# JdeRobot/slam-SDVL

Hardware: AMD Instinct MI355X
Metric: tracked frames/sec (640x480, 5-lvl pyr, ~200 feats) (higher is better)
Workload: dtype u8/f32/f64

## Files before the change

### slam-sdvl_amd/csrc/sdvl_detect.hip

```cpp
#include <atomic>

#include "sdvl_internal.h"
#include "sdvl_wave.h"

namespace {

constexpr int kPyrTW = 32, kPyrTH = 8;

struct PyrJob {
  const uint8_t *src;
  uint8_t *dst;
  int sw, sh, dw, dh;
};

__device__ __forceinline__ int reflect101_clamped(int p, int n) {
  if (p < 0) p = -p;
  if (p >= n) p = 2 * n - 2 - p;
  return min(max(p, 0), n - 1);
}

template <int kPyrTW, int kPyrTH>
__global__ __launch_bounds__(kPyrTW * kPyrTH / 4) void pyr_down_kernel(const PyrJob *__restrict__ jobs, int n_jobs, int gx, int gy) {
  constexpr int kThreads = kPyrTW * kPyrTH / 4;
  constexpr int kPyrSH = 2 * kPyrTH + 3;
  constexpr int kPyrSWW = kPyrTW / 2 + 2;
  constexpr int kPyrPitch = (kPyrSWW + 1) * 4;
  const auto sync = [] {
    if (kThreads == 64) wave_sync();
    else __syncthreads();
  };
  __shared__ uint32_t s_srcw[kPyrSH * (kPyrSWW + 1)];
  __shared__ __attribute__((aligned(8))) uint16_t s_h[kPyrSH][kPyrTW];
  const int id = blockIdx.x, per_frame = gx * gy;
  const int slot = id >> 3;
  const int bz = (slot / per_frame) * 8 + (id & 7);
  if (bz >= n_jobs) return;
  const int tq = slot % per_frame;
  const int by = tq / gx, bx = tq - by * gx;
  const PyrJob job = jobs[bz];
  const int tx0 = bx * kPyrTW, ty0 = by * kPyrTH;
  if (tx0 >= job.dw || ty0 >= job.dh) return;
  const int tid = threadIdx.x;
  uint8_t *s_bytes = reinterpret_cast<uint8_t *>(s_srcw);
  const int xb = 2 * tx0 - 4;
  const int nx = min(kPyrTW, job.dw - tx0), ny = min(kPyrTH, job.dh - ty0);
  const int rows = 2 * ny + 3, last_byte = 2 * nx + 4;
  if ((job.sw & 3) == 0 && (reinterpret_cast<uintptr_t>(job.src) & 3u) == 0) {
    const int words_row = job.sw >> 2, w0 = xb >> 2;
    const int nwords = last_byte / 4 + 1;
    constexpr int kRowLanes = (kPyrSWW + 3) / 4, kRowsPerRound = kThreads / kRowLanes;
    if (words_row >= 4) {
      const int lr = tid / kRowLanes, lq = tid - lr * kRowLanes;
      const int first = w0 + 4 * lq;
      const int s = min(max(first, 0), words_row - 4);
      const int col0 = s - w0;
      if (lr < kRowsPerRound && 4 * lq < nwords) {
        for (int r = lr; r < rows; r += kRowsPerRound) {
          const int sy = reflect101_clamped(2 * ty0 - 2 + r, job.sh);
          const __attribute__((address_space(1))) uint32_t *srcw = (const __attribute__((address_space(1))) uint32_t *)job.src;
          const __attribute__((address_space(1))) uint32_t *pw = srcw + static_cast<uint32_t>(sy * words_row + s);
          const uint32_t v[4] = {pw[0], pw[1], pw[2], pw[3]};
          uint32_t *dst = &s_srcw[r * (kPyrSWW + 1)];
#pragma unroll
          for (int k = 0; k < 4; k++) {
            const int c = col0 + k;
            if (c >= 0 && c < nwords) dst[c] = v[k];
          }
        }
      }
    } else
    for (int idx = tid; idx < rows * kPyrSWW; idx += kThreads) {
      const int r = idx / kPyrSWW, c = idx - r * kPyrSWW;
      if (c >= nwords) continue;
      const int sy = reflect101_clamped(2 * ty0 - 2 + r, job.sh);
      const int wi = min(max(w0 + c, 0), words_row - 1);
      s_srcw[r * (kPyrSWW + 1) + c] = reinterpret_cast<const uint32_t *>(job.src + static_cast<size_t>(sy) * job.sw)[wi];
    }
    sync();
    if (tid < rows && (xb < 0 || xb + last_byte >= job.sw)) {
      uint8_t *row = s_bytes + tid * kPyrPitch;
      if (xb < 0) {
        row[2] = row[6];
        row[3] = row[5];
      }
      for (int b = max(2, job.sw - xb); b <= last_byte; b++) row[b] = row[max(reflect101_clamped(xb + b, job.sw) - xb, 0)];
    }
  } else {
    const int ncols = last_byte - 1;
    for (int idx = tid; idx < rows * ncols; idx += kThreads) {
      const int r = idx / ncols, c = idx - r * ncols;
      const int sy = reflect101_clamped(2 * ty0 - 2 + r, job.sh);
      const int sx = reflect101_clamped(2 * tx0 - 2 + c, job.sw);
      s_bytes[r * kPyrPitch + 2 + c] = job.src[static_cast<size_t>(sy) * job.sw + sx];
    }
  }
  sync();
  typedef unsigned short u16x2 __attribute__((ext_vector_type(2)));
  for (int idx = tid; idx < rows * (kPyrTW / 2); idx += kThreads) {
    const int r = idx / (kPyrTW / 2), xp = idx - r * (kPyrTW / 2);
    if (2 * xp < nx) {
      const uint32_t *w = &s_srcw[r * (kPyrSWW + 1) + xp];
      const uint32_t w0 = w[0], w1 = w[1], w2 = w[2];
      const uint32_t hx = __builtin_amdgcn_udot4(w1, 0x00010406u, __builtin_amdgcn_udot4(w0, 0x04010000u, 0u, false), false);
      const uint32_t hx1 = __builtin_amdgcn_udot4(w2, 0x00000001u, __builtin_amdgcn_udot4(w1, 0x04060401u, 0u, false), false);
      const uint32_t h = hx | (hx1 << 16);
      *reinterpret_cast<uint32_t *>(&s_h[r][2 * xp]) = __builtin_bit_cast(uint32_t, h);
    }
  }
  sync();
  {
    const int y = tid / (kPyrTW / 4), x = (tid % (kPyrTW / 4)) * 4;
    const int oy = ty0 + y, ox = tx0 + x;
    if (oy < job.dh && ox < job.dw) {
      u16x2 a01 = {0, 0}, a23 = {0, 0};
#pragma unroll
      for (int t = 0; t < 5; t++) {
        const unsigned short wg = (t == 0 || t == 4) ? 1 : (t == 2 ? 6 : 4);
        const u16x2 wgt = {wg, wg};
        const uint2 hv = *reinterpret_cast<const uint2 *>(&s_h[2 * y + t][x]);
        a01 += wgt * __builtin_bit_cast(u16x2, hv.x);
        a23 += wgt * __builtin_bit_cast(u16x2, hv.y);
      }
      const u16x2 half = {128, 128};
      a01 = (a01 + half) >> 8;
      a23 = (a23 + half) >> 8;
      int acc[4] = {a01.x, a01.y, a23.x, a23.y};
      uint8_t *d = job.dst + static_cast<size_t>(oy) * job.dw + ox;
      if (ox + 3 < job.dw && (reinterpret_cast<uintptr_t>(job.dst) & 3u) == 0 && (job.dw & 3) == 0) {
        __attribute__((address_space(1))) uint32_t *dstw = (__attribute__((address_space(1))) uint32_t *)job.dst;
        dstw[static_cast<uint32_t>(oy * job.dw + ox) >> 2] = __builtin_amdgcn_perm(__builtin_bit_cast(uint32_t, a23), __builtin_bit_cast(uint32_t, a01), 0x06040200u);
      } else {
#pragma unroll
        for (int k = 0; k < 4; k++)
          if (ox + k < job.dw) d[k] = static_cast<uint8_t>(acc[k]);
      }
    }
  }
}

struct FastLevels {
  int n_levels;
  int cell_begin[SDVL_MAX_LEVELS + 1];
  int wcells[SDVL_MAX_LEVELS];
  int cell_size, margin, threshold;
  int dense_num;
};

struct __attribute__((aligned(16))) CellGeo {
  uint32_t xy;
  uint32_t wh;
  int32_t level;
  int32_t pair_inv;
};

struct FastJob {
  const uint8_t *level[4];
  int lw[4], lh[4];
  uint32_t *cell_kps;
  int32_t *cell_counts;
};


constexpr int kTile = 32;
constexpr int kPitchW = 12;
constexpr int kPadRows = 3;

__device__ __forceinline__ bool ring_run9(uint32_t m) {
  const uint32_t M = m | (m << 16);
  uint32_t r = M & (M >> 1);
  r &= (r >> 2);
  r &= (r >> 4);
  r &= (M >> 8);
  return (r & 0xFFFFu) != 0;
}

__device__ __forceinline__ int byte_of(uint32_t w0, uint32_t w1, uint32_t w2, int i) {
  return static_cast<int>(((i < 4 ? w0 : (i < 8 ? w1 : w2)) >> (8 * (i & 3))) & 0xFFu);
}

__device__ __forceinline__ bool fast_compass_pass(int v, int p_dn, int p_rt, int p_up, int p_lf, int t) {
  const int hi = v + t, lo = v - t;
  const bool b0 = p_dn > hi, b4 = p_rt > hi, b8 = p_up > hi, b12 = p_lf > hi;
  const bool d0 = p_dn < lo, d4 = p_rt < lo, d8 = p_up < lo, d12 = p_lf < lo;
  return (b0 && b4) || (b4 && b8) || (b8 && b12) || (b12 && b0) || (d0 && d4) || (d4 && d8) || (d8 && d12) || (d12 && d0);
}

#define SDVL_MIN2(a, b) min((a), (b))
#define SDVL_MAX2(a, b) max((a), (b))

__device__ __forceinline__ int fast_corner_best(const uint8_t *tile, int pitch_bytes, int t) {
  const int v = tile[0];
#define SDVL_E(K, DX, DY) const int e##K = static_cast<int>(tile[(DY) * pitch_bytes + (DX)]);
  SDVL_E(0, 0, 3) SDVL_E(1, 1, 3) SDVL_E(2, 2, 2) SDVL_E(3, 3, 1) SDVL_E(4, 3, 0) SDVL_E(5, 3, -1) SDVL_E(6, 2, -2) SDVL_E(7, 1, -3)
  SDVL_E(8, 0, -3) SDVL_E(9, -1, -3) SDVL_E(10, -2, -2) SDVL_E(11, -3, -1) SDVL_E(12, -3, 0) SDVL_E(13, -3, 1) SDVL_E(14, -2, 2) SDVL_E(15, -1, 3)
#undef SDVL_E
#define SDVL_MIN3(a, b, c) min(min((a), (b)), (c))
#define SDVL_MAX3(a, b, c) max(max((a), (b)), (c))
#define SDVL_W3(K, A, B, C) const int n##K = SDVL_MIN3(e##A, e##B, e##C), x##K = SDVL_MAX3(e##A, e##B, e##C);
  SDVL_W3(0, 0, 1, 2) SDVL_W3(1, 1, 2, 3) SDVL_W3(2, 2, 3, 4) SDVL_W3(3, 3, 4, 5) SDVL_W3(4, 4, 5, 6) SDVL_W3(5, 5, 6, 7)
  SDVL_W3(6, 6, 7, 8) SDVL_W3(7, 7, 8, 9) SDVL_W3(8, 8, 9, 10) SDVL_W3(9, 9, 10, 11) SDVL_W3(10, 10, 11, 12) SDVL_W3(11, 11, 12, 13)
  SDVL_W3(12, 12, 13, 14) SDVL_W3(13, 13, 14, 15) SDVL_W3(14, 14, 15, 0) SDVL_W3(15, 15, 0, 1)
#undef SDVL_W3
#define SDVL_W9(K, A, B, C) const int N##K = SDVL_MIN3(n##A, n##B, n##C), X##K = SDVL_MAX3(x##A, x##B, x##C);
  SDVL_W9(0, 0, 3, 6) SDVL_W9(1, 1, 4, 7) SDVL_W9(2, 2, 5, 8) SDVL_W9(3, 3, 6, 9) SDVL_W9(4, 4, 7, 10) SDVL_W9(5, 5, 8, 11)
  SDVL_W9(6, 6, 9, 12) SDVL_W9(7, 7, 10, 13) SDVL_W9(8, 8, 11, 14) SDVL_W9(9, 9, 12, 15) SDVL_W9(10, 10, 13, 0) SDVL_W9(11, 11, 14, 1)
  SDVL_W9(12, 12, 15, 2) SDVL_W9(13, 13, 0, 3) SDVL_W9(14, 14, 1, 4) SDVL_W9(15, 15, 2, 5)
#undef SDVL_W9
  const int max_n = SDVL_MAX3(SDVL_MAX3(N0, N1, N2), SDVL_MAX3(N3, N4, N5), SDVL_MAX3(SDVL_MAX3(N6, N7, N8), SDVL_MAX3(N9, N10, N11), SDVL_MAX3(N12, N13, SDVL_MAX2(N14, N15))));
  const int min_x = SDVL_MIN3(SDVL_MIN3(X0, X1, X2), SDVL_MIN3(X3, X4, X5), SDVL_MIN3(SDVL_MIN3(X6, X7, X8), SDVL_MIN3(X9, X10, X11), SDVL_MIN3(X12, X13, SDVL_MIN2(X14, X15))));
#undef SDVL_MIN3
#undef SDVL_MAX3
  return max(max(t, v - min_x), max_n - v);
}


constexpr int kPitchHW = 20;

typedef _Float16 h2 __attribute__((ext_vector_type(2)));
__device__ __forceinline__ h2 pk_min3(h2 a, h2 b, h2 c) {
  h2 d;
  asm("v_pk_minimum3_f16 %0, %1, %2, %3" : "=v"(d) : "v"(a), "v"(b), "v"(c));
  return d;
}
__device__ __forceinline__ h2 pk_max3(h2 a, h2 b, h2 c) {
  h2 d;
  asm("v_pk_maximum3_f16 %0, %1, %2, %3" : "=v"(d) : "v"(a), "v"(b), "v"(c));
  return d;
}
__device__ __forceinline__ h2 as_h2(uint32_t w) { return __builtin_bit_cast(h2, w); }
__device__ __forceinline__ h2 mid_h2(uint32_t hi, uint32_t lo) { return as_h2(__builtin_amdgcn_alignbit(hi, lo, 16)); }

struct PairRing {
  uint32_t a1, a2, b1, b2, c0, c1, c2, c3, d0, d1, d2, d3, z0, z1, z2, z3, u0, u3, l0, l3;
};

__device__ __forceinline__ h2 fast_pair_best_ring(const PairRing &q, h2 t2) {
  const h2 e0 = mid_h2(q.a2, q.a1), e1 = as_h2(q.a2), e2 = mid_h2(q.c3, q.c2), e3 = as_h2(q.u3), e4 = as_h2(q.z3), e5 = as_h2(q.l3),
           e6 = mid_h2(q.d3, q.d2), e7 = as_h2(q.b2), e8 = mid_h2(q.b2, q.b1), e9 = as_h2(q.b1), e10 = mid_h2(q.d1, q.d0), e11 = as_h2(q.l0),
           e12 = as_h2(q.z0), e13 = as_h2(q.u0), e14 = mid_h2(q.c1, q.c0), e15 = as_h2(q.a1);
  const h2 v = mid_h2(q.z2, q.z1);
#define SDVL_W3(K, A, B, C) const h2 n##K = pk_min3(e##A, e##B, e##C), x##K = pk_max3(e##A, e##B, e##C);
  SDVL_W3(0, 0, 1, 2) SDVL_W3(1, 1, 2, 3) SDVL_W3(2, 2, 3, 4) SDVL_W3(3, 3, 4, 5) SDVL_W3(4, 4, 5, 6) SDVL_W3(5, 5, 6, 7)
  SDVL_W3(6, 6, 7, 8) SDVL_W3(7, 7, 8, 9) SDVL_W3(8, 8, 9, 10) SDVL_W3(9, 9, 10, 11) SDVL_W3(10, 10, 11, 12) SDVL_W3(11, 11, 12, 13)
  SDVL_W3(12, 12, 13, 14) SDVL_W3(13, 13, 14, 15) SDVL_W3(14, 14, 15, 0) SDVL_W3(15, 15, 0, 1)
#undef SDVL_W3
#define SDVL_W9(K, A, B, C) const h2 N##K = pk_min3(n##A, n##B, n##C), X##K = pk_max3(x##A, x##B, x##C);
  SDVL_W9(0, 0, 3, 6) SDVL_W9(1, 1, 4, 7) SDVL_W9(2, 2, 5, 8) SDVL_W9(3, 3, 6, 9) SDVL_W9(4, 4, 7, 10) SDVL_W9(5, 5, 8, 11)
  SDVL_W9(6, 6, 9, 12) SDVL_W9(7, 7, 10, 13) SDVL_W9(8, 8, 11, 14) SDVL_W9(9, 9, 12, 15) SDVL_W9(10, 10, 13, 0) SDVL_W9(11, 11, 14, 1)
  SDVL_W9(12, 12, 15, 2) SDVL_W9(13, 13, 0, 3) SDVL_W9(14, 14, 1, 4) SDVL_W9(15, 15, 2, 5)
#undef SDVL_W9
  const h2 max_n = pk_max3(pk_max3(pk_max3(N0, N1, N2), pk_max3(N3, N4, N5), pk_max3(N6, N7, N8)),
                           pk_max3(pk_max3(N9, N10, N11), pk_max3(N12, N13, N14), N15), N15);
  const h2 min_x = pk_min3(pk_min3(pk_min3(X0, X1, X2), pk_min3(X3, X4, X5), pk_min3(X6, X7, X8)),
                           pk_min3(pk_min3(X9, X10, X11), pk_min3(X12, X13, X14), X15), X15);
  return pk_max3(t2, v - min_x, max_n - v);
}

__device__ __forceinline__ void fast_quad_best(const uint32_t *w, h2 t2, h2 *best_a, h2 *best_b) {
  const auto w2 = [w](int dy, int k) { return *reinterpret_cast<const uint2 *>(&w[(dy + 3) * kPitchHW + k]); };
  const auto w1 = [w](int dy, int k) { return w[(dy + 3) * kPitchHW + k]; };
  const uint32_t a1 = w1(3, 1), b1 = w1(-3, 1);
  const uint2 a23 = w2(3, 2), b23 = w2(-3, 2);
  const uint2 c01 = w2(2, 0), c23 = w2(2, 2), d01 = w2(-2, 0), d23 = w2(-2, 2), z01 = w2(0, 0), z23 = w2(0, 2), u01 = w2(1, 0), l01 = w2(-1, 0);
  const uint32_t c4 = w1(2, 4), d4 = w1(-2, 4), z4 = w1(0, 4), u3 = w1(1, 3), u4 = w1(1, 4), l3 = w1(-1, 3), l4 = w1(-1, 4);
  const PairRing qa = {a1, a23.x, b1, b23.x, c01.x, c01.y, c23.x, c23.y, d01.x, d01.y, d23.x, d23.y, z01.x, z01.y, z23.x, z23.y, u01.x, u3, l01.x, l3};
  const PairRing qb = {a23.x, a23.y, b23.x, b23.y, c01.y, c23.x, c23.y, c4, d01.y, d23.x, d23.y, d4, z01.y, z23.x, z23.y, z4, u01.y, u4, l01.y, l4};
  *best_a = fast_pair_best_ring(qa, t2);
  *best_b = fast_pair_best_ring(qb, t2);
}

__device__ __forceinline__ int wave_rank4(uint32_t flags, int *wave_total) {
  int below = 0, total = 0;
#pragma unroll
  for (int k = 0; k < 4; k++) {
    const unsigned long long m = __ballot((flags >> k) & 1u);
    below += __builtin_amdgcn_mbcnt_hi(static_cast<uint32_t>(m >> 32), __builtin_amdgcn_mbcnt_lo(static_cast<uint32_t>(m), 0));
    total += __popcll(m);
  }
  *wave_total = total;
  return below;
}

typedef __attribute__((address_space(1))) uint32_t *FcGlobalWords;
__device__ __forceinline__ FcGlobalWords fc_slot(FcGlobalWords base, int pos) {
  return (FcGlobalWords)((__attribute__((address_space(1))) char *)base + (static_cast<uint32_t>(pos) << 2));
}

constexpr int kFcDenseWords = (kTile + 2 * kPadRows) * kPitchHW + (kTile + 2) * kPitchHW;
constexpr int kFcSparseWords = (kTile + 2 * kPadRows) * kPitchW + (kTile + 2) * kPitchW + kTile * kTile / 2;
static_assert(kFcSparseWords <= kFcDenseWords, "the sparse layout lives inside the dense one");
static_assert(((kTile + 2 * kPadRows) * kPitchHW * 4) % 16 == 0, "the half score plane is cleared with 16-byte stores");

// ... 729 lines not shown
#pragma unroll
    for (int o = 1; o < 64; o <<= 1) {
      const int t = __shfl_up(incl, o, 64);
      if (lane >= o) incl += t;
    }
    const int nfts = __shfl(incl, 63, 64);
    int dst = incl - mine;
    int n = -1;
    if (nfts <= lv.spill_cap[l]) {
      const bool fits = nfts <= lv.fts_cap[l];
      uint32_t *spill = job.spill + lv.spill_off[l];
      if (fits) {
        uint32_t *v = lists[l];
        for (int c = c_lo; c < c_hi; c++) {
          const int len = job.cell_newlen[cbeg + c];
          const uint32_t *src = job.cell_kps + static_cast<size_t>(cbeg + c) * lv.kp_stride;
          for (int k = 0; k < len; k++) v[dst++] = src[k];
        }
        wave_sync();
        n = nfts;
        if (nfts > lv.quota[l]) {
          uint16_t *Ls = reinterpret_cast<uint16_t *>(v + lv.fts_cap[l]);
          n = group_retain_best<64, uint16_t>(v, nfts, lv.quota[l], Ls, Ls + lv.fts_cap[l], lane, 0);
        }
      } else {
        uint32_t *v = spill;
        for (int c = c_lo; c < c_hi; c++) {
          const int len = job.cell_newlen[cbeg + c];
          const uint32_t *src = job.cell_kps + static_cast<size_t>(cbeg + c) * lv.kp_stride;
          for (int k = 0; k < len; k++) v[dst++] = src[k];
        }
        wave_sync();
        n = nfts;
        if (nfts > lv.quota[l]) {
          uint16_t *Ls = reinterpret_cast<uint16_t *>(v + lv.spill_cap[l]);
          n = group_retain_best<64, uint16_t>(v, nfts, lv.quota[l], Ls, Ls + lv.spill_cap[l], lane, 0);
        }
        wave_sync();
      }
      if (lane == 0) s_n[l] = fits ? n : (n | 0x40000000);
    } else if (lane == 0) {
      s_n[l] = -1;
    }
  }
  for (int c = tid; c < cells; c += 256) s_hist[c] = 0;
  __syncthreads();
  int lvl_off[5];
  bool bad = false;
  lvl_off[0] = 0;
  for (int l = 0; l < lv.n_levels; l++) {
    const int raw = s_n[l];
    if (raw < 0) { bad = true; lvl_off[l + 1] = lvl_off[l]; continue; }
    if (raw & 0x40000000) lists[l] = job.spill + lv.spill_off[l];
    lvl_off[l + 1] = lvl_off[l] + (raw & 0x3FFFFFFF);
  }
  if (lvl_off[lv.n_levels] > job.corner_cap) bad = true;
  const int n = bad ? 0 : lvl_off[lv.n_levels];
  if (tid == 0) {
    const int total = bad ? -1 : n;
    job.corner_hdr[0] = n;
    job.corner_hdr[1] = total;
    if (batch_counts) batch_counts[blockIdx.x] = total;
    if (host_counts) host_counts[blockIdx.x] = total;
  }
  if (bad) {
    for (int c = tid; c <= cells; c += 256)
      if (cells > 0) job.bin_start[c] = 0;
    return;
  }
  int4 *out = reinterpret_cast<int4 *>(job.corner_hdr + 4);
  const auto cell_of = [&](uint32_t v, int l) {
    const int x = min(static_cast<int>(v & 0xFFF) << l, job.lw[0] - 1), y = min(static_cast<int>((v >> 12) & 0xFFF) << l, job.lh[0] - 1);
    return (y >> 5) * job.bin_gw + (x >> 5);
  };
  for (int l = 0; l < lv.n_levels; l++) {
    const int nl = lvl_off[l + 1] - lvl_off[l];
    const uint32_t *v = lists[l];
    for (int k = tid; k < nl; k += 256) {
      const uint32_t e = v[k];
      out[lvl_off[l] + k] = make_int4(static_cast<int>(e & 0xFFF), static_cast<int>((e >> 12) & 0xFFF), l, 0);
      if (cells > 0) atomicAdd(&s_hist[cell_of(e, l)], 1);
    }
  }
  if (cells <= 0) return;
  __syncthreads();
  const int per = (cells + 255) / 256, c0 = min(cells, tid * per), c1 = min(cells, c0 + per);
  int sum = 0;
  for (int c = c0; c < c1; c++) sum += s_hist[c];
  s_part[tid] = sum;
  __syncthreads();
  if (tid < 64) {
    const int a0 = s_part[4 * tid], a1 = s_part[4 * tid + 1], a2 = s_part[4 * tid + 2], a3 = s_part[4 * tid + 3];
    int incl = a0 + a1 + a2 + a3;
    const int own = incl;
#pragma unroll
    for (int o = 1; o < 64; o <<= 1) {
      const int t = __shfl_up(incl, o, 64);
      if (tid >= o) incl += t;
    }
    const int ex = incl - own;
    s_part[4 * tid] = ex;
    s_part[4 * tid + 1] = ex + a0;
    s_part[4 * tid + 2] = ex + a0 + a1;
    s_part[4 * tid + 3] = ex + a0 + a1 + a2;
  }
  __syncthreads();
  {
    int run = s_part[tid];
    for (int c = c0; c < c1; c++) {
      const int v = s_hist[c];
      job.bin_start[c] = run;
      s_hist[c] = run;
      run += v;
    }
    if (tid == 0) job.bin_start[cells] = n;
  }
  __syncthreads();
  for (int l = 0; l < lv.n_levels; l++) {
    const int nl = lvl_off[l + 1] - lvl_off[l];
    const uint32_t *v = lists[l];
    for (int k = tid; k < nl; k += 256) {
      const uint32_t e = v[k];
      const int slot = atomicAdd(&s_hist[cell_of(e, l)], 1);
      job.bin_entries[slot] = make_uint2((e & 0xFFFFFFu) | (static_cast<uint32_t>(l) << 24), static_cast<uint32_t>(lvl_off[l] + k));
    }
  }
}

__global__ __launch_bounds__(64) void retain_best_kernel(uint32_t *v, int len, int n_points, int *out_len, int form) {
  __shared__ uint32_t s_v[kSelFts];
  __shared__ uint16_t s_l[kSelFts], s_r[kSelFts];
  if (form == 2 && len <= SDVL_CELL_KP_CAP) {
    uint8_t *gl = reinterpret_cast<uint8_t *>(s_l), *gr = reinterpret_cast<uint8_t *>(s_r);
    for (int i = threadIdx.x; i < len; i += 64) s_v[i] = v[i];
    wave_sync();
    if (threadIdx.x >= kSelGroup && threadIdx.x < 2 * kSelGroup) {
      const int n = group_retain_best<kSelGroup, uint8_t>(s_v, len, n_points, gl, gr, threadIdx.x - kSelGroup, kSelGroup);
      if (threadIdx.x == kSelGroup) *out_len = n;
    }
    wave_sync();
    for (int i = threadIdx.x; i < len; i += 64) v[i] = s_v[i];
  } else if (form == 3 && len <= kSelFts) {
    for (int i = threadIdx.x; i < len; i += 64) s_v[i] = v[i];
    wave_sync();
    const int n = group_retain_best<64, uint16_t>(s_v, len, n_points, s_l, s_r, threadIdx.x, 0);
    if (threadIdx.x == 0) *out_len = n;
    wave_sync();
    for (int i = threadIdx.x; i < len; i += 64) v[i] = s_v[i];
  } else if (threadIdx.x == 0) {
    *out_len = sel_retain_best(v, len, n_points);
  }
}

}

extern "C" {

int sdvl_pyramid_build(sdvl_ctx *ctx, int n, sdvl_frame *const *frames) {
  if (!ctx || n < 0 || (n > 0 && !frames)) return SDVL_ERR_INVALID;
  if (n == 0) return SDVL_OK;
  int levels = frames[0]->v.levels;
  for (int i = 0; i < n; i++) {
    SDVL_REQUIRE(ctx, frames[i] != nullptr, "null frame");
    SDVL_REQUIRE(ctx, frames[i]->v.levels == levels && frames[i]->width == frames[0]->width && frames[i]->height == frames[0]->height,
                 "frames of one batch must share size and pyramid depth");
  }
  if (levels < 2) return SDVL_OK;
  const size_t bytes = sizeof(PyrJob) * n * (levels - 1);
  void *hs = nullptr, *dsx = nullptr;
  int rc = sdvl_stage_alloc(ctx, bytes, &hs, &dsx);
  if (rc) return rc;
  PyrJob *hj = static_cast<PyrJob *>(hs);
  for (int l = 1; l < levels; l++)
    for (int i = 0; i < n; i++) {
      const FrameView &v = frames[i]->v;
      hj[(l - 1) * n + i] = PyrJob{v.level[l - 1], v.level[l], v.lw[l - 1], v.lh[l - 1], v.lw[l], v.lh[l]};
    }
  SDVL_HIP_CHECK(ctx, sdvl_push(ctx, dsx, hj, bytes));
  for (int l = 1; l < levels; l++) {
    const FrameView &v = frames[0]->v;
    const int gx = (v.lw[l] + kPyrTW - 1) / kPyrTW, gy = (v.lh[l] + kPyrTH - 1) / kPyrTH;
    const dim3 grid = dim3(static_cast<unsigned>(gx) * gy * ((n + 7) / 8 * 8), 1, 1);
    SDVL_LAUNCH(ctx, "pyr_down", (pyr_down_kernel<kPyrTW, kPyrTH>), grid, dim3(64), static_cast<const PyrJob *>(dsx) + (l - 1) * n, n, gx, gy);
  }
  SDVL_HIP_CHECK(ctx, hipGetLastError());
  return SDVL_OK;
}

int sdvl_cell_kp_cap(int cell_size) {
  if (cell_size < 8 || cell_size > SDVL_MAX_CELL_SIZE) return 0;
  if (cell_size <= 32) return SDVL_CELL_KP_CAP;
  const int half = (cell_size - 6 + 1) / 2;
  return half * half;
}

struct DetectSlot {
  size_t counts_off, newlen_off, kps_off, spill_off, bytes;
};
static DetectSlot detect_slot_layout(int total_cells, int kp_cap, size_t spill_words) {
  DetectSlot L;
  sdvl_layout lay;
  L.counts_off = lay.take<int32_t>(static_cast<size_t>(total_cells) + 1).off;
  L.newlen_off = lay.take<int32_t>(total_cells).off;
  L.kps_off = lay.take<uint32_t>(static_cast<size_t>(kp_cap) * static_cast<size_t>(total_cells)).off;
  L.spill_off = lay.take<uint32_t>(spill_words).off;
  L.bytes = lay.bytes();
  return L;
}

static int sel_spill_cap(int ncells) { return std::max(kSelFts, std::min(65536, (8 * ncells + 63) / 64 * 64)); }
static int detect_scratch(sdvl_ctx *ctx, int n, const DetectSlot &L, uint8_t **base) {
  const int rc = sdvl_ensure(ctx, &ctx->d_detect, &ctx->d_detect_bytes, L.bytes * static_cast<size_t>(n), false);
  if (rc) return rc;
  *base = static_cast<uint8_t *>(ctx->d_detect);
  return SDVL_OK;
}

static int fast_cells_dense_num() {
  static const int v = [] {
    const char *e = getenv("SDVL_FAST_DENSE_NUM");
    const int n = e ? atoi(e) : 16;
    return n < 0 ? 0 : (n > 64 ? 64 : n);
  }();
  return v;
}

struct DetectPlan {
  FastLevels lv;
  SelLevels sl;
  int total_cells, kp_cap;
  int n_slices;
  int sel_form;
  size_t pack_lds;
  DetectSlot slot;
};

static DetectPlan detect_plan(const int *lw, const int *lh, const sdvl_detect_params *p, int nfeatures) {
  DetectPlan pl;
  memset(&pl, 0, sizeof(pl));
  FastLevels &lv = pl.lv;
  SelLevels &sl = pl.sl;
  const int cs = p->cell_size, margin = p->margin;
  lv.n_levels = sl.n_levels = p->max_fast_levels;
  lv.cell_size = sl.cell_size = cs;
  lv.margin = sl.margin = margin;
  lv.threshold = p->fast_threshold < 0 ? 0 : (p->fast_threshold > 255 ? 255 : p->fast_threshold);
  lv.dense_num = fast_cells_dense_num();
  pl.kp_cap = sl.kp_stride = sdvl_cell_kp_cap(cs);
  const double scale = 1.2;
  double factor = 1.0, val = 0.0;
  for (int i = 0; i < lv.n_levels; i++) { val += factor; factor /= scale; }
  int levelfeatures = nfeatures < 0 ? 0 : static_cast<int>(nfeatures / val);
  int max_cells = 0;
  for (int l = 0; l < lv.n_levels; l++) {
    lv.wcells[l] = sl.wcells[l] = (lw[l] + cs - 1) / cs;
    sl.hcells[l] = (lh[l] + cs - 1) / cs;
    max_cells = std::max(max_cells, sl.wcells[l] * sl.hcells[l]);
  }
  pl.sel_form = cs > kTile ? 2 : (max_cells > kSelMaxCells ? 1 : 0);
  const int sel_cells_per_wave = pl.sel_form == 2 ? 1 : kSelCellsPerWave;
  size_t spill_words = 0;
  for (int l = 0; l < lv.n_levels; l++) {
    const int ncells = sl.wcells[l] * sl.hcells[l];
    lv.cell_begin[l] = sl.cell_begin[l] = pl.total_cells;
    pl.total_cells += ncells;
    sl.quota[l] = levelfeatures;
    levelfeatures = static_cast<int>(levelfeatures / scale);
    int rows_run = 0, cols_run = 0;
    for (int ci = 0; ci < sl.hcells[l]; ci++) rows_run += std::min(lh[l] - margin, ci * cs + cs) > std::max(margin, ci * cs) ? 1 : 0;
    for (int cj = 0; cj < sl.wcells[l]; cj++) cols_run += std::min(lw[l] - margin, cj * cs + cs) > std::max(margin, cj * cs) ? 1 : 0;
    sl.not_run[l] = ncells - rows_run * cols_run;
    sl.slice_begin[l] = pl.n_slices;
    pl.n_slices += (ncells + sel_cells_per_wave - 1) / sel_cells_per_wave;
    sl.fts_cap[l] = std::min(kSelFts, ((sl.quota[l] + ncells) * 3 / 2 + 63) / 64 * 64);
    pl.pack_lds += static_cast<size_t>(sl.fts_cap[l]) * 8;
    sl.spill_cap[l] = sel_spill_cap(ncells);
    sl.spill_off[l] = static_cast<int>(spill_words);
    spill_words += 2 * static_cast<size_t>(sl.spill_cap[l]);
  }
  lv.cell_begin[lv.n_levels] = sl.cell_begin[sl.n_levels] = pl.total_cells;
  sl.slice_begin[sl.n_levels] = pl.n_slices;
  pl.slot = detect_slot_layout(pl.total_cells, pl.kp_cap, spill_words);
  return pl;
}

static bool detect_plan_size(int width, int height, const sdvl_detect_params *p, DetectPlan *pl) {
  if (!p || p->cell_size <= 0 || p->max_fast_levels < 1 || p->max_fast_levels > 4) return false;
  int lw[4], lh[4];
  for (int l = 0, w = width, h = height; l < p->max_fast_levels; l++, w /= 2, h /= 2) {
    lw[l] = w;
    lh[l] = h;
  }
  *pl = detect_plan(lw, lh, p, -1);
  return true;
}

int sdvl_fast_num_cells(int width, int height, const sdvl_detect_params *p, int *cells_per_level, int *total) {
  DetectPlan pl;
  if (!detect_plan_size(width, height, p, &pl)) return SDVL_ERR_INVALID;
  for (int l = 0; l < pl.lv.n_levels && cells_per_level; l++) cells_per_level[l] = pl.lv.cell_begin[l + 1] - pl.lv.cell_begin[l];
  if (total) *total = pl.total_cells;
  return SDVL_OK;
}

int64_t sdvl_detect_scratch_bytes(int width, int height, const sdvl_detect_params *p) {
  DetectPlan pl;
  if (!detect_plan_size(width, height, p, &pl) || pl.kp_cap == 0) return -1;
  return static_cast<int64_t>(pl.slot.bytes);
}

static int detect_plan_frames(sdvl_ctx *ctx, int n, sdvl_frame *const *frames, const sdvl_detect_params *p, int nfeatures, DetectPlan *pl) {
  SDVL_REQUIRE(ctx, p->cell_size >= 8 && p->cell_size <= SDVL_MAX_CELL_SIZE, "cell_size must be in [8,64]");
  SDVL_REQUIRE(ctx, p->max_fast_levels >= 1 && p->max_fast_levels <= 4, "max_fast_levels must be in [1,4]");
  SDVL_REQUIRE(ctx, p->margin >= 0, "margin must not be negative");
  for (int i = 0; i < n; i++)
    SDVL_REQUIRE(ctx, frames[i] && frames[i]->width == frames[0]->width && frames[i]->height == frames[0]->height &&
                          frames[i]->v.levels == frames[0]->v.levels,
                 "frames of one batch must share size and pyramid depth");
  SDVL_REQUIRE(ctx, p->max_fast_levels <= frames[0]->v.levels, "max_fast_levels exceeds the pyramid depth");
  *pl = detect_plan(frames[0]->v.lw, frames[0]->v.lh, p, nfeatures);
  for (int l = 0; l < pl->lv.n_levels; l++)
    SDVL_REQUIRE(ctx, pl->lv.cell_begin[l + 1] - pl->lv.cell_begin[l] <= SDVL_MAX_LEVEL_CELLS,
                 "too many cells in one level (8192: at most 3840x2160 at cell 32)");
  return SDVL_OK;
}

static FastJob fast_job(const DetectPlan &pl, const sdvl_frame *f, uint8_t *slot) {
  FastJob j;
  memset(&j, 0, sizeof(j));
  for (int l = 0; l < pl.lv.n_levels; l++) {
    j.level[l] = f->v.level[l];
    j.lw[l] = f->v.lw[l];
    j.lh[l] = f->v.lh[l];
  }
  j.cell_kps = reinterpret_cast<uint32_t *>(slot + pl.slot.kps_off);
  j.cell_counts = reinterpret_cast<int32_t *>(slot + pl.slot.counts_off);
// ... 296 lines not shown
```

### slam-sdvl_amd/csrc/sdvl_layout.h

```cpp
#ifndef SDVL_LAYOUT_H_
#define SDVL_LAYOUT_H_

#include <stddef.h>
#include <stdint.h>

inline size_t sdvl_align256(size_t v) { return (v + 255) / 256 * 256; }

template <typename T>
struct sdvl_part {
  size_t off = 0, count = 0;
  size_t bytes() const { return sizeof(T) * count; }
  T *in(void *base) const { return reinterpret_cast<T *>(static_cast<uint8_t *>(base) + off); }
  const T *cin(const void *base) const { return reinterpret_cast<const T *>(static_cast<const uint8_t *>(base) + off); }
};

struct sdvl_layout {
  size_t size = 0;
  template <typename T>
  sdvl_part<T> take(size_t count) {
    const sdvl_part<T> p{size, count};
    size = sdvl_align256(size + p.bytes());
    return p;
  }
  size_t bytes() const { return size; }
};

#endif
```

Baseline: 468,300.

## Add strip-walking pyramid downsample kernel that reuses vertical halo rows

Adds a pyramid-downsample kernel in which each 64-thread block walks several vertically stacked output tiles. The 3-row horizontal-sum halo is carried between tiles in a two-slot LDS ring, and the next tile's source rows are loaded into registers while the current tile is computed. This cuts redundant halo reads and per-tile block launch overhead when the grid is large. A heuristic enables it only when the strip grid would still hold many waves; otherwise, or when environment overrides or alignment checks say so, it falls back to the old kernel. Fewer blocks means less parallelism, and the longer serial loop per block adds sync points.

```diff
diff --git a/slam-sdvl_amd/csrc/sdvl_detect.hip b/slam-sdvl_amd/csrc/sdvl_detect.hip
--- a/slam-sdvl_amd/csrc/sdvl_detect.hip
+++ b/slam-sdvl_amd/csrc/sdvl_detect.hip
@@ -138,6 +138,139 @@
   }
 }
 
+__global__ __launch_bounds__(64) void pyr_down_strip_kernel(const PyrJob *__restrict__ jobs, int n_jobs, int gx, int gys, int tiles) {
+  using L = sdvl_pyr_strip_lds;
+  constexpr int kRowLanes = (L::kRowWords + 3) / 4, kRowsPerRound = 64 / kRowLanes;
+  static_assert(L::kNewRows <= 2 * kRowsPerRound && L::kHalo <= kRowsPerRound, "a tile's rows come in with two loads per lane");
+  __shared__ uint32_t s_srcw[L::kNewRows * L::kPitchWords];
+  __shared__ __attribute__((aligned(8))) uint16_t s_h[L::kRingRows][L::kTW];
+  const int id = blockIdx.x, per_frame = gx * gys;
+  const int slot = id >> 3;
+  const int bz = (slot / per_frame) * 8 + (id & 7);
+  if (bz >= n_jobs) return;
+  const int tq = slot % per_frame;
+  const int by = tq / gx, bx = tq - by * gx;
+  const PyrJob job = jobs[bz];
+  const int tx0 = bx * L::kTW, ty_first = by * tiles * L::kTH;
+  if (tx0 >= job.dw || ty_first >= job.dh) return;
+  const int ty_end = min(job.dh, ty_first + tiles * L::kTH);
+  const int tid = threadIdx.x;
+  const int xb = 2 * tx0 - 4;
+  const int nx = min(L::kTW, job.dw - tx0), last_byte = 2 * nx + 4;
+  const int words_row = job.sw >> 2, w0 = xb >> 2, nwords = last_byte / 4 + 1;
+  const int base_row = 2 * ty_first - 2;
+  const int lr = tid / kRowLanes, lq = tid - lr * kRowLanes;
+  const int s = min(max(w0 + 4 * lq, 0), words_row - 4);
+  const int col0 = s - w0;
+  const bool loader = lr < kRowsPerRound && 4 * lq < nwords;
+  const bool mend = xb < 0 || xb + last_byte >= job.sw;
+  const __attribute__((address_space(1))) uint32_t *srcw = (const __attribute__((address_space(1))) uint32_t *)job.src;
+  const auto load_row = [&](int row, bool inside, uint32_t (&v)[4]) {
+    const int sy = inside ? row : reflect101_clamped(row, job.sh);
+    const __attribute__((address_space(1))) uint32_t *pw = srcw + static_cast<uint32_t>(sy * words_row + s);
+    v[0] = pw[0], v[1] = pw[1], v[2] = pw[2], v[3] = pw[3];
+  };
+  const auto stage_row = [&](int r, const uint32_t (&v)[4]) {
+    uint32_t *dst = &s_srcw[r * L::kPitchWords];
+#pragma unroll
+    for (int k = 0; k < 4; k++) {
+      const int c = col0 + k;
+      if (c >= 0 && c < nwords) dst[c] = v[k];
+    }
+  };
+  uint32_t va[4], vb[4];
+  const auto issue = [&](int row0, int nrows) {
+    const bool inside = row0 >= 0 && row0 + nrows <= job.sh;
+    if (loader && lr < nrows) load_row(row0 + lr, inside, va);
+    if (loader && kRowsPerRound + lr < nrows) load_row(row0 + kRowsPerRound + lr, inside, vb);
+  };
+  const auto commit = [&](int nrows) {
+    if (loader && lr < nrows) stage_row(lr, va);
+    if (loader && kRowsPerRound + lr < nrows) stage_row(kRowsPerRound + lr, vb);
+  };
+  const auto mend_rows = [&](int nrows) {
+    if (mend && tid < nrows) {
+      uint8_t *row = reinterpret_cast<uint8_t *>(s_srcw) + tid * (L::kPitchWords * 4);
+      if (xb < 0) {
+        row[2] = row[6];
+        row[3] = row[5];
+      }
+      for (int b = max(2, job.sw - xb); b <= last_byte; b++) row[b] = row[max(reflect101_clamped(xb + b, job.sw) - xb, 0)];
+    }
+  };
+  const auto hsum_rows = [&](int nrows, int ring0, bool odd) {
+    constexpr int kRowsPerPass = 64 / (L::kTW / 2);
+    const int xp = tid % (L::kTW / 2);
+#pragma unroll
+    for (int r0 = 0; r0 < L::kNewRows; r0 += kRowsPerPass) {
+      const int r = r0 + tid / (L::kTW / 2);
+      if (r < nrows && 2 * xp < nx) {
+        const uint32_t *w = &s_srcw[r * L::kPitchWords + xp];
+        const uint32_t q0 = w[0], q1 = w[1], q2 = w[2];
+        const uint32_t hx = __builtin_amdgcn_udot4(q1, 0x00010406u, __builtin_amdgcn_udot4(q0, 0x04010000u, 0u, false), false);
+        const uint32_t hx1 = __builtin_amdgcn_udot4(q2, 0x00000001u, __builtin_amdgcn_udot4(q1, 0x04060401u, 0u, false), false);
+        *reinterpret_cast<uint32_t *>(&s_h[ring0 + r][2 * xp]) = hx | (hx1 << 16);
+        if (r0 + kRowsPerPass > L::kNewRows - L::kHalo && odd && r >= L::kNewRows - L::kHalo) *reinterpret_cast<uint32_t *>(&s_h[r - (L::kNewRows - L::kHalo)][2 * xp]) = hx | (hx1 << 16);
+      }
+    }
+  };
+  typedef unsigned short u16x2 __attribute__((ext_vector_type(2)));
+  const bool dst_words = (reinterpret_cast<uintptr_t>(job.dst) & 3u) == 0 && (job.dw & 3) == 0;
+  const int y = tid / (L::kTW / 4), ox = tx0 + (tid % (L::kTW / 4)) * 4;
+
+  int ty0 = ty_first, ny = min(L::kTH, ty_end - ty0);
+  {
+    uint32_t vh[4];
+    if (loader && lr < L::kHalo) load_row(base_row + lr, false, vh);
+    issue(base_row + L::kHalo, 2 * ny);
+    if (loader && lr < L::kHalo) stage_row(lr, vh);
+  }
+  wave_sync();
+  mend_rows(L::kHalo);
+  wave_sync();
+  hsum_rows(L::kHalo, 0, false);
+  wave_sync();
+  for (int t = 0;; t++) {
+    commit(2 * ny);
+    wave_sync();
+    const int ty_next = ty0 + L::kTH, ny_next = min(L::kTH, ty_end - ty_next);
+    if (ny_next > 0) issue(base_row + L::kNewRows * (t + 1) + L::kHalo, 2 * ny_next);
+    mend_rows(2 * ny);
+    wave_sync();
+    const int ring_t = (t & 1) * L::kNewRows;
+    hsum_rows(2 * ny, ring_t + L::kHalo, (t & 1) != 0);
+    wave_sync();
+    if (y < ny && ox < job.dw) {
+      u16x2 a01 = {0, 0}, a23 = {0, 0};
+#pragma unroll
+      for (int k = 0; k < 5; k++) {
+        const unsigned short wg = (k == 0 || k == 4) ? 1 : (k == 2 ? 6 : 4);
+        const u16x2 wgt = {wg, wg};
+        const uint2 hv = *reinterpret_cast<const uint2 *>(&s_h[ring_t + 2 * y + k][ox - tx0]);
+        a01 += wgt * __builtin_bit_cast(u16x2, hv.x);
+        a23 += wgt * __builtin_bit_cast(u16x2, hv.y);
+      }
+      const u16x2 half = {128, 128};
+      a01 = (a01 + half) >> 8;
+      a23 = (a23 + half) >> 8;
+      const int oy = ty0 + y;
+      if (ox + 3 < job.dw && dst_words) {
+        __attribute__((address_space(1))) uint32_t *dstw = (__attribute__((address_space(1))) uint32_t *)job.dst;
+        dstw[static_cast<uint32_t>(oy * job.dw + ox) >> 2] = __builtin_amdgcn_perm(__builtin_bit_cast(uint32_t, a23), __builtin_bit_cast(uint32_t, a01), 0x06040200u);
+      } else {
+        const int acc[4] = {a01.x, a01.y, a23.x, a23.y};
+        uint8_t *d = job.dst + static_cast<size_t>(oy) * job.dw + ox;
+#pragma unroll
+        for (int k = 0; k < 4; k++)
+          if (ox + k < job.dw) d[k] = static_cast<uint8_t>(acc[k]);
+      }
+    }
+    if (ny_next <= 0) break;
+    ty0 = ty_next, ny = ny_next;
+    wave_sync();
+  }
+}
+
 struct FastLevels {
   int n_levels;
   int cell_begin[SDVL_MAX_LEVELS + 1];
@@ -1173,6 +1306,13 @@
   }
 }
 
+constexpr int kPyrStripRows = 5, kPyrStripMaxTiles = 8, kPyrStripMinWaves = 4096;
+int pyr_strip_tiles(int n, int gx, int gy) {
+  const int tiles = std::min(kPyrStripMaxTiles, gy / kPyrStripRows);
+  if (tiles < 2) return 0;
+  return static_cast<long long>(n) * gx * ((gy + tiles - 1) / tiles) >= kPyrStripMinWaves ? tiles : 0;
+}
+
 }
 
 extern "C" {
@@ -1198,11 +1338,30 @@
       hj[(l - 1) * n + i] = PyrJob{v.level[l - 1], v.level[l], v.lw[l - 1], v.lh[l - 1], v.lw[l], v.lh[l]};
     }
   SDVL_HIP_CHECK(ctx, sdvl_push(ctx, dsx, hj, bytes));
+  const bool no_strips = getenv("SDVL_PYR_NO_STRIPS") != nullptr;
+  const char *forced = getenv("SDVL_PYR_STRIP_TILES");
   for (int l = 1; l < levels; l++) {
+    int forced_tiles = -1;
+    if (forced) {
+      forced_tiles = atoi(forced);
+      const char *comma = strchr(forced, ',');
+      if (comma) forced = comma + 1;
+    }
     const FrameView &v = frames[0]->v;
     const int gx = (v.lw[l] + kPyrTW - 1) / kPyrTW, gy = (v.lh[l] + kPyrTH - 1) / kPyrTH;
-    const dim3 grid = dim3(static_cast<unsigned>(gx) * gy * ((n + 7) / 8 * 8), 1, 1);
-    SDVL_LAUNCH(ctx, "pyr_down", (pyr_down_kernel<kPyrTW, kPyrTH>), grid, dim3(64), static_cast<const PyrJob *>(dsx) + (l - 1) * n, n, gx, gy);
+    const PyrJob *jobs = static_cast<const PyrJob *>(dsx) + (l - 1) * n;
+    int tiles = no_strips ? 0 : (forced_tiles >= 0 ? forced_tiles : pyr_strip_tiles(n, gx, gy));
+    bool aligned = (v.lw[l - 1] & 3) == 0 && v.lw[l - 1] >= 16;
+    for (int i = 0; i < n && aligned && tiles > 0; i++) aligned = (reinterpret_cast<uintptr_t>(frames[i]->v.level[l - 1]) & 3u) == 0;
+    if (tiles > 0 && aligned) {
+      tiles = std::min(tiles, gy);
+      const int gys = (gy + tiles - 1) / tiles;
+      const dim3 grid = dim3(static_cast<unsigned>(gx) * gys * ((n + 7) / 8 * 8), 1, 1);
+      SDVL_LAUNCH(ctx, "pyr_down", pyr_down_strip_kernel, grid, dim3(64), jobs, n, gx, gys, tiles);
+    } else {
+      const dim3 grid = dim3(static_cast<unsigned>(gx) * gy * ((n + 7) / 8 * 8), 1, 1);
+      SDVL_LAUNCH(ctx, "pyr_down", (pyr_down_kernel<kPyrTW, kPyrTH>), grid, dim3(64), jobs, n, gx, gy);
+    }
   }
   SDVL_HIP_CHECK(ctx, hipGetLastError());
   return SDVL_OK;
diff --git a/slam-sdvl_amd/csrc/sdvl_layout.h b/slam-sdvl_amd/csrc/sdvl_layout.h
--- a/slam-sdvl_amd/csrc/sdvl_layout.h
+++ b/slam-sdvl_amd/csrc/sdvl_layout.h
@@ -25,4 +25,15 @@
   size_t bytes() const { return size; }
 };
 
+struct sdvl_pyr_strip_lds {
+  static constexpr int kTW = 32, kTH = 8;
+  static constexpr int kHalo = 3, kNewRows = 2 * kTH;
+  static constexpr int kRowWords = kTW / 2 + 2, kPitchWords = kRowWords + 1;
+  static constexpr int kRingRows = 2 * kNewRows + kHalo;
+  static constexpr size_t stage_bytes = sizeof(uint32_t) * kNewRows * kPitchWords;
+  static constexpr size_t ring_bytes = sizeof(uint16_t) * kRingRows * kTW;
+  static constexpr size_t bytes = stage_bytes + ring_bytes;
+};
+static_assert(sdvl_pyr_strip_lds::bytes <= 5 * 1024, "32 waves per CU");
+
 #endif
```

Result: slower. 459,800 (-1.8%).
